# qcraftai/gedepth

Hardware: AMD Instinct MI355X
Metric: training img/s (whole node), KITTI-shaped 352x1120 synthetic batches (higher is better)
Workload: dtype bf16; 1 GPU; depthformer_swint_v: DepthFormer-SwinT + GEDepth-Vanilla, 352x1120, 8 img/GPU, full train step; global_batch=8, parallelism=dp1, allreduce_dtype=fp32, layout=nhwc, window_attention=bf16 mfma, params=53516992, hip_graph=off

## Files before the change

gedepth_amd/csrc/conv1x1_bn.hip:

```cpp
#include "common.h"

#define CB_K 64
#define CB_LD 72
#define CB_GRAM (65 * CB_K)
#define CB_GRAM_WG 256

__device__ __forceinline__ int cb_row(int r, int hi) { return (r & 3) + 8 * (r >> 2) + 4 * hi; }

__global__ void __launch_bounds__(256) conv1x1_gram_k(const bf16_t* __restrict__ x, long rows, float* __restrict__ partial) {
  __shared__ __attribute__((aligned(16))) bf16_t stage_all[4][64 * CB_LD];
  __shared__ float red[CB_GRAM];
  const int lane = threadIdx.x & 63, wv = threadIdx.x >> 6, hi = lane >> 5;
  bf16_t* stage = stage_all[wv];
  ge_f32x16 acc[2][2], sum[2];
#pragma unroll
  for (int i = 0; i < 16; ++i) { acc[0][0][i] = 0.f; acc[0][1][i] = 0.f; acc[1][0][i] = 0.f; acc[1][1][i] = 0.f; sum[0][i] = 0.f; sum[1][i] = 0.f; }
  const ge_bf16x8 ones = {(__bf16)1.f, (__bf16)1.f, (__bf16)1.f, (__bf16)1.f, (__bf16)1.f, (__bf16)1.f, (__bf16)1.f, (__bf16)1.f};
  const int tr_row = hi * 8 + ((lane & 15) >> 2), tr_col = ((lane >> 4) & 1) * 16 + (lane & 3) * 4;
  const long nblk = (rows + 63) / 64;
  for (long blk = (long)blockIdx.x * 4 + wv; blk < nblk; blk += (long)gridDim.x * 4) {
    uint4 R[8];
#pragma unroll
    for (int i = 0; i < 8; ++i) {
      const int idx = i * 64 + lane;
// ... 310 lines not shown
  if (sl == 0) {
    a = (sm[0][j] + sm[1][j]) + (sm[2][j] + sm[3][j]);
    const bf16_t r = f2bf(a);
    Wd[(long)j * (Cout + CB_K) + Cout + i] = r;
    b += (float)(gram[CB_K * CB_K + j] / n) * (a - bf2f(r));
  }
  b = ge_wave_sum(b);
  if (j == 0) sc[sl] = b;
  __syncthreads();
  if (threadIdx.x == 0) c0v[i] = (sc[0] + sc[1]) + (sc[2] + sc[3]);
}

__global__ void __launch_bounds__(256) conv1x1_bn_dgrad_k(const bf16_t* __restrict__ g, const bf16_t* __restrict__ x, const bf16_t* __restrict__ Wd,
                                                          const float* __restrict__ c0, bf16_t* __restrict__ dx, long rows, int Cout) {
  extern __shared__ __attribute__((aligned(16))) bf16_t wl[];
  const int KP = Cout + CB_K, LD = KP + 8, ppr = KP / 8;
  for (int idx = threadIdx.x; idx < CB_K * ppr; idx += 256) {
    const int r = idx / ppr, pc = idx - r * ppr;
    *(uint4*)(wl + r * LD + pc * 8) = *(const uint4*)(Wd + (long)r * KP + pc * 8);
  }
  __syncthreads();
  const int lane = threadIdx.x & 63, wv = threadIdx.x >> 6, hi = lane >> 5, n = lane & 31;
  float c0r[2][16];
#pragma unroll
  for (int mt = 0; mt < 2; ++mt)
#pragma unroll
    for (int r = 0; r < 16; ++r) c0r[mt][r] = c0[mt * 32 + cb_row(r, hi)];
  const bf16_t* wa = wl + n * LD + hi * 8;
  const long ntile = (rows + 31) / 32, tstep = (long)gridDim.x * 4;
  const int nch = Cout / 128;
  ge_bf16x8 Fa[8], Fb[8], Fx[4];
#define CB_ROWPTR(T_) (((T_) * 32 + n < rows) ? (T_) * 32 + n : rows - 1)
#define CB_LOADG(F_, T_, C_) { const bf16_t* gr_ = g + CB_ROWPTR(T_) * Cout + (C_) * 128 + hi * 8; _Pragma("unroll") for (int s_ = 0; s_ < 8; ++s_) F_[s_] = *(const ge_bf16x8*)(gr_ + s_ * 16); }
#define CB_MMA(F_, C_)                                                                                                         \
  _Pragma("unroll") for (int s_ = 0; s_ < 8; ++s_) {                                                                           \
    const ge_bf16x8 w0_ = *(const ge_bf16x8*)(wa + ((C_) * 8 + s_) * 16), w1_ = *(const ge_bf16x8*)(wa + 32 * LD + ((C_) * 8 + s_) * 16); \
    acc0 = __builtin_amdgcn_mfma_f32_32x32x16_bf16(w0_, F_[s_], acc0, 0, 0, 0);                                                 \
    acc1 = __builtin_amdgcn_mfma_f32_32x32x16_bf16(w1_, F_[s_], acc1, 0, 0, 0);                                                 \
  }
  long tile = (long)blockIdx.x * 4 + wv;
  if (tile < ntile) CB_LOADG(Fa, tile, 0)
  for (; tile < ntile; tile += tstep) {
    {
      const bf16_t* xr = x + CB_ROWPTR(tile) * CB_K + hi * 8;
#pragma unroll
      for (int s = 0; s < 4; ++s) Fx[s] = *(const ge_bf16x8*)(xr + s * 16);
    }
    ge_f32x16 acc0, acc1;
#pragma unroll
    for (int i = 0; i < 16; ++i) { acc0[i] = 0.f; acc1[i] = 0.f; }
    for (int c = 0; c < nch; c += 2) {
      if (c + 1 < nch) CB_LOADG(Fb, tile, c + 1)
      CB_MMA(Fa, c)
      if (c + 2 < nch) CB_LOADG(Fa, tile, c + 2)
      else if (tile + tstep < ntile) CB_LOADG(Fa, tile + tstep, 0)
      if (c + 1 < nch) CB_MMA(Fb, c + 1)
    }
#pragma unroll
    for (int s = 0; s < 4; ++s) {
      const ge_bf16x8 w0 = *(const ge_bf16x8*)(wa + Cout + s * 16), w1 = *(const ge_bf16x8*)(wa + 32 * LD + Cout + s * 16);
      acc0 = __builtin_amdgcn_mfma_f32_32x32x16_bf16(w0, Fx[s], acc0, 0, 0, 0);
      acc1 = __builtin_amdgcn_mfma_f32_32x32x16_bf16(w1, Fx[s], acc1, 0, 0, 0);
    }
    const long row = tile * 32 + n;
    if (row < rows) {
      bf16_t* o = dx + row * CB_K + 4 * hi;
#pragma unroll
      for (int r4 = 0; r4 < 4; ++r4) {
        uint2 v0, v1;
        v0.x = ge_pack_bf16x2(acc0[4 * r4] + c0r[0][4 * r4], acc0[4 * r4 + 1] + c0r[0][4 * r4 + 1]);
        v0.y = ge_pack_bf16x2(acc0[4 * r4 + 2] + c0r[0][4 * r4 + 2], acc0[4 * r4 + 3] + c0r[0][4 * r4 + 3]);
        v1.x = ge_pack_bf16x2(acc1[4 * r4] + c0r[1][4 * r4], acc1[4 * r4 + 1] + c0r[1][4 * r4 + 1]);
        v1.y = ge_pack_bf16x2(acc1[4 * r4 + 2] + c0r[1][4 * r4 + 2], acc1[4 * r4 + 3] + c0r[1][4 * r4 + 3]);
        *(uint2*)(o + 8 * r4) = v0;
        *(uint2*)(o + 32 + 8 * r4) = v1;
      }
    }
  }
#undef CB_ROWPTR
#undef CB_LOADG
#undef CB_MMA
}

static inline bool cb_ok(int Cin, int Cout) { return Cin == CB_K && Cout > 0 && Cout % 128 == 0 && Cout <= 2048; }

extern "C" size_t ge_conv1x1_bn_workspace(int Cin, int Cout) {
  if (!cb_ok(Cin, Cout)) return 0;
  const size_t a = (size_t)CB_GRAM_WG * CB_GRAM * sizeof(float), b = (size_t)1024 * Cout * sizeof(float);
  return a > b ? a : b;
}

extern "C" int ge_conv1x1_bn_stats(const void* x, long rows, int Cin, const void* w, int Cout, const float* gamma, const float* beta,
                                   float* running_mean, float* running_var, float eps, float momentum, double* gram, float* save_mean,
                                   float* save_rstd, float* coef, void* workspace, void* stream) {
  if (!x || !w || !gamma || !beta || !gram || !save_mean || !save_rstd || !coef || !workspace || rows <= 0) return GE_ERR_BAD_ARG;
  if (!cb_ok(Cin, Cout) || (((uintptr_t)x | (uintptr_t)w) & 15)) return GE_ERR_UNSUPPORTED;
  hipStream_t s = ge_stream(stream);
  const long nblk = (rows + 63) / 64;
  const int nb = (int)(nblk < 4L * CB_GRAM_WG ? (nblk + 3) / 4 : CB_GRAM_WG);
  conv1x1_gram_k<<<nb, 256, 0, s>>>((const bf16_t*)x, rows, (float*)workspace);
  GE_LAUNCH_CHECK();
  conv1x1_partials_reduce_k<double><<<(CB_GRAM + 31) / 32, 256, 0, s>>>((const float*)workspace, nb, CB_GRAM, gram);
  GE_LAUNCH_CHECK();
  conv1x1_bn_finalize_k<<<(Cout + 3) / 4, 256, 0, s>>>(gram, (const bf16_t*)w, gamma, beta, save_mean, save_rstd, running_mean, running_var, coef,
                                                       Cout, (double)rows, eps, momentum);
  GE_LAUNCH_CHECK();
  return GE_OK;
}

extern "C" int ge_conv1x1_bn_act_fwd(const void* x, const void* w, const float* coef, const float* pos, void* y, void* q, int B, long HW, int Cin,
                                     int Cout, float slope, void* stream) {
  if (!x || !w || !coef || !y || B <= 0 || HW <= 0 || (!pos) != (!q)) return GE_ERR_BAD_ARG;
  if (!cb_ok(Cin, Cout) || (((uintptr_t)x | (uintptr_t)w | (uintptr_t)y | (uintptr_t)q | (uintptr_t)pos) & 15)) return GE_ERR_UNSUPPORTED;
  const int cus = ge_cu_count();
  if (!cus) return GE_ERR_BAD_ARG;
  hipStream_t s = ge_stream(stream);
  const long ntile = ((HW + 31) / 32) * B;
#ifndef CB_WGS_PER_CU
#define CB_WGS_PER_CU 4
#endif
  long gx = (long)cus * CB_WGS_PER_CU;
  if (gx > ntile) gx = ntile;
  gx = (gx + 7) / 8 * 8;
  const dim3 grid((unsigned)gx, (unsigned)((Cout / 128 + 3) / 4));
  if (pos) conv1x1_bn_act_k<true><<<grid, 256, 0, s>>>((const bf16_t*)x, (const bf16_t*)w, coef, pos, (bf16_t*)y, (bf16_t*)q, HW, B, Cout, slope);
  else conv1x1_bn_act_k<false><<<grid, 256, 0, s>>>((const bf16_t*)x, (const bf16_t*)w, coef, nullptr, (bf16_t*)y, nullptr, HW, B, Cout, slope);
  GE_LAUNCH_CHECK();
  return GE_OK;
}

extern "C" int ge_conv1x1_bn_bwd_mask(const void* dy1, long ld1, const void* dy2, long ld2, const void* y, void* g, float* colsum, void* workspace,
                                      long rows, int C, float slope, void* stream) {
  if ((!dy1 && !dy2) || !y || !g || !colsum || !workspace || rows <= 0 || C <= 0) return GE_ERR_BAD_ARG;
  if (C % 8 || C > 2048 || (dy1 && ld1 % 8) || (dy2 && ld2 % 8) || (((uintptr_t)dy1 | (uintptr_t)dy2 | (uintptr_t)y | (uintptr_t)g) & 15)) return GE_ERR_UNSUPPORTED;
  hipStream_t s = ge_stream(stream);
  const int lpr = C / 8;
  if (lpr > 256) return GE_ERR_UNSUPPORTED;
  const int rpi = 256 / lpr;
  const unsigned nb = ge_blocks(rows, rpi * 8, 1024);
  float* part = (float*)workspace;
#define CB_MASK(A_, B_) conv1x1_bn_mask_k<A_, B_><<<nb, 256, 0, s>>>((const bf16_t*)dy1, ld1, (const bf16_t*)dy2, ld2, (const bf16_t*)y, (bf16_t*)g, part, C, rows, lpr, rpi, slope)
  if (dy1 && dy2) CB_MASK(true, true);
  else if (dy1) CB_MASK(true, false);
  else CB_MASK(false, true);
#undef CB_MASK
  GE_LAUNCH_CHECK();
  conv1x1_partials_reduce_k<float><<<(C + 31) / 32, 256, 0, s>>>(part, (int)nb, C, colsum);
  GE_LAUNCH_CHECK();
  return GE_OK;
}

extern "C" int ge_conv1x1_bn_bwd_finalize(const float* GT, const float* colsum, const double* gram, const void* w, const float* gamma,
                                          const float* save_mean, const float* save_rstd, long rows, int Cin, int Cout, float* dgamma, float* dbeta,
                                          float* dW, void* Wd, float* c0, float* scratch, void* stream) {
  if (!GT || !colsum || !gram || !w || !gamma || !save_mean || !save_rstd || !dgamma || !dbeta || !dW || !Wd || !c0 || !scratch || rows <= 0) return GE_ERR_BAD_ARG;
  if (!cb_ok(Cin, Cout)) return GE_ERR_UNSUPPORTED;
  hipStream_t s = ge_stream(stream);
  conv1x1_bn_bwd_finalize_k<<<(Cout + 3) / 4, 256, 0, s>>>(GT, colsum, gram, (const bf16_t*)w, gamma, save_mean, save_rstd, dgamma, dbeta, dW, (bf16_t*)Wd,
                                                           scratch, scratch + Cout, Cout, (double)rows);
  GE_LAUNCH_CHECK();
  conv1x1_bn_bwd_a2_k<<<CB_K, 256, 0, s>>>((const bf16_t*)w, scratch, scratch + Cout, gram, (bf16_t*)Wd, c0, Cout, (double)rows);
  GE_LAUNCH_CHECK();
  return GE_OK;
}

extern "C" int ge_conv1x1_bn_dgrad(const void* g, const void* x, const void* Wd, const float* c0, void* dx, long rows, int Cin, int Cout, void* stream) {
  if (!g || !x || !Wd || !c0 || !dx || rows <= 0) return GE_ERR_BAD_ARG;
  if (!cb_ok(Cin, Cout) || Cout > 1024 || (((uintptr_t)g | (uintptr_t)x | (uintptr_t)Wd | (uintptr_t)dx) & 15)) return GE_ERR_UNSUPPORTED;
  const int cus = ge_cu_count();
  if (!cus) return GE_ERR_BAD_ARG;
  const size_t smem = (size_t)CB_K * (Cout + CB_K + 8) * sizeof(bf16_t);
  static bool attr_set = false;
  if (!attr_set) {
    if (hipFuncSetAttribute((const void*)conv1x1_bn_dgrad_k, hipFuncAttributeMaxDynamicSharedMemorySize, 160 * 1024) != hipSuccess) return GE_ERR_UNSUPPORTED;
    attr_set = true;
  }
  const long ntile = (rows + 31) / 32;
  long wgs = (long)cus * (smem <= 78 * 1024 ? 2 : 1);
  if (wgs > (ntile + 3) / 4) wgs = (ntile + 3) / 4;
  conv1x1_bn_dgrad_k<<<(unsigned)wgs, 256, smem, ge_stream(stream)>>>((const bf16_t*)g, (const bf16_t*)x, (const bf16_t*)Wd, c0, (bf16_t*)dx, rows, Cout);
  GE_LAUNCH_CHECK();
  return GE_OK;
}
```

gedepth_amd/hip.py:

```python
import ctypes
import os
import re

import torch

_HERE = os.path.dirname(os.path.abspath(__file__))
LIB_PATH = os.environ.get('GE_LIB') or os.path.join(_HERE, 'csrc', 'libgedepth_hip.so')
HEADERS = {'SIGNATURES': 'gedepth_hip.h', 'EVAL_SIGNATURES': 'gedepth_eval.h', 'DDAD_SIGNATURES': 'gedepth_ddad.h',
           'CLOUD_SIGNATURES': 'gedepth_cloud.h', 'GROUND_SIGNATURES': 'gedepth_ground.h'}
EXTRA_HEADERS = {'BATCH_SIGNATURES': 'gedepth_batch.h'}
SCENE_HEADERS = {'SCENE_SIGNATURES': 'gedepth_scene.h'}
STRATA_HEADERS = {'STRATA_SIGNATURES': 'gedepth_strata.h'}
GE_F32, GE_BF16 = 0, 1
GE_COLORIZE_VMIN_DATA, GE_COLORIZE_VMAX_DATA, GE_COLORIZE_EQUAL = 1, 2, 4

_SCALARS = {'int': ctypes.c_int, 'long': ctypes.c_long, 'float': ctypes.c_float, 'double': ctypes.c_double, 'size_t': ctypes.c_size_t,
            'uint64_t': ctypes.c_ulonglong, 'unsigned long long': ctypes.c_ulonglong}
_DECL = re.compile(r'\b(int|size_t)\s+(ge_\w+)\s*\(([^()]*)\)\s*;')


def parse_header(text):
    text = re.sub(r'/\*.*?\*/|//[^\n]*', ' ', text, flags=re.S)
    sigs = {}
    for res, name, params in _DECL.findall(text):
        args = []
        for p in ([] if params.strip() == 'void' else params.split(',')):
            if '*' in p:
                args.append(ctypes.c_void_p)
                continue
            ctype = ' '.join(w for w in p.split()[:-1] if w != 'const')
            if ctype not in _SCALARS:
                raise TypeError(f'{name}: parameter "{" ".join(p.split())}" has a type the ctypes binding does not map')
            args.append(_SCALARS[ctype])
        sigs[name] = (_SCALARS[res], args)
    stray = set(re.findall(r'\b(ge_\w+)\s*\(', text)) - set(sigs)
    if stray:
        raise TypeError(f'cannot parse the declaration of {", ".join(sorted(stray))}')
    return sigs


for _table, _header in {**HEADERS, **EXTRA_HEADERS, **SCENE_HEADERS, **STRATA_HEADERS}.items():
    with open(os.path.join(os.path.dirname(_HERE), 'include', _header)) as _fh:
        globals()[_table] = parse_header(_fh.read())

_lib = None


class HipLibraryError(RuntimeError):
    pass


def lib():
    global _lib
    if _lib is None:
        if not os.path.isfile(LIB_PATH):
            raise HipLibraryError(
                f'{LIB_PATH} is missing: the gfx950 HIP kernels are not built. '
                f'Run gedepth_amd/csrc/build.sh (hipcc --offload-arch=gfx950). There is no CPU/eager fallback.')
        handle = ctypes.CDLL(LIB_PATH)
        for table in (*HEADERS, *EXTRA_HEADERS, *SCENE_HEADERS, *STRATA_HEADERS):
            for name, (res, args) in globals()[table].items():
                fn = getattr(handle, name)
                fn.restype, fn.argtypes = res, args
        _lib = handle
        if os.environ.get('GE_MSDA_MODE'):
            handle.ge_msda_mode(int(os.environ['GE_MSDA_MODE']))
    return _lib


def is_built():
    return os.path.isfile(LIB_PATH)


def check(code, what):
    if code != 0:
        raise RuntimeError(f'{what} failed with code {code} '
                           f'({"bad argument" if code == 10001 else "unsupported" if code == 10002 else "hipError_t"})')


def call(name, *args):
    code = getattr(_lib or lib(), name)(*args)
    if code:
        check(code, name)


def dtype_code(t):
    if t.dtype == torch.float32:
        return GE_F32
    if t.dtype == torch.bfloat16:
        return GE_BF16
    raise TypeError(f'gedepth_amd kernels take float32 or bfloat16 tensors, got {t.dtype}')


def ptr(t, dtype=None, name='tensor'):
    if t is None:
        return None
    if not t.is_cuda:
        raise RuntimeError(f'{name}: gedepth_amd ops run on MI355X only; got a {t.device} tensor '
                           '(the CPU oracle lives in oracle/ and is test infrastructure)')
    if not t.is_contiguous():
        raise RuntimeError(f'{name} must be contiguous')
    if dtype is not None and t.dtype != dtype:
        raise TypeError(f'{name} must be {dtype}, got {t.dtype}')
    return t.data_ptr()


def stream():
    return torch.cuda.current_stream().cuda_stream
```

gedepth_amd/kernels.py:

```python
import ctypes
import os

import torch

from . import hip

_f32 = torch.float32


def _c(t):
    return t if t.is_contiguous() else t.contiguous()


class _Profiler:

    def __init__(self):
        self.on, self.records, self.stage_bytes = False, {}, {}

    def enable(self):
        self.on, self.records, self.stage_bytes = True, {}, {}
        hip.lib().ge_msda_bwd_timing(1)

    def disable(self):
        self.on = False
# ... 1423 lines not shown
                hip.ptr(y), hip.ptr(stats[0]), hip.ptr(stats[1]), hip.ptr(running_mean, _f32), hip.ptr(running_var, _f32), hip.ptr(ws), N, C, H * W,
                eps, momentum, slope, hip.dtype_code(x), hip.stream())
        ctx.save_for_backward(x, y, w, stats)
        ctx.slope = slope
        return y

    @staticmethod
    def backward(ctx, dy):
        x, y, w, stats = ctx.saved_tensors
        N, C, H, W = x.shape
        dx = torch.empty_like(x)
        dwb = torch.empty(2, C, device=x.device, dtype=_f32)
        ws = torch.empty(int(hip.lib().ge_nhwc_workspace(C, 2) if ctx.cl else hip.lib().ge_bn_workspace(C)), device=x.device, dtype=torch.uint8)
        if ctx.cl:
            dy = _cl(dy.to(x.dtype))
            _launch(f'bn_act_nhwc_bwd[{N}x{C}x{H}x{W} {_tag(x)}]', 5 * x.numel() * _es(x), 'ge_bn_act_nhwc_bwd', _raw_ptr(dy, 'dy'), None,
                    _raw_ptr(x, 'x'), hip.ptr(w), hip.ptr(y, _f32), hip.ptr(stats[0]), hip.ptr(stats[1]), _raw_ptr(dx, 'dx'), hip.ptr(dwb[0]),
                    hip.ptr(dwb[1]), hip.ptr(ws), N * H * W, C, ctx.slope, hip.dtype_code(x), hip.stream())
            return dx, dwb[0], dwb[1], None, None, None, None, None
        dy = _c(dy.to(x.dtype))
        _launch(f'bn_act_bwd[{N}x{C}x{H}x{W} {_tag(x)}]', 7 * x.numel() * _es(x), 'ge_bn_act_bwd', hip.ptr(dy), hip.ptr(y), hip.ptr(x), hip.ptr(w),
                hip.ptr(stats[0]), hip.ptr(stats[1]), hip.ptr(dx), hip.ptr(dwb[0]), hip.ptr(dwb[1]), hip.ptr(ws), N, C, H * W, ctx.slope,
                hip.dtype_code(x), hip.stream())
        return dx, dwb[0], dwb[1], None, None, None, None, None


def bn_act(x, bn, slope=0.0):
    y = _BNAct.apply(x, bn.weight, bn.bias, bn.running_mean, bn.running_var, float(bn.eps), float(bn.momentum), float(slope))
    bn.num_batches_tracked.add_(1)
    return y


class _Conv1x1BNActPos(torch.autograd.Function):

    @staticmethod
    def forward(ctx, x, weight, gamma, beta, running_mean, running_var, pos_rows, eps, momentum, slope):
        from .mmrt.optim import lowp
        lib = hip.lib()
        B, Cin, H, W = x.shape
        Cout = weight.shape[0]
        HW, rows = H * W, B * H * W
        wc = lowp(weight, torch.bfloat16).detach().reshape(Cout, Cin)
        g32, b32 = _c(gamma.detach().to(_f32)), _c(beta.detach().to(_f32))
        dev = x.device
        ws = torch.empty(int(lib.ge_conv1x1_bn_workspace(Cin, Cout)), device=dev, dtype=torch.uint8)
        gram = torch.empty(65 * Cin, device=dev, dtype=torch.float64)
        stats = torch.empty(2, Cout, device=dev, dtype=_f32)
        coef = torch.empty(2, Cout, device=dev, dtype=_f32)
        y = torch.empty((B, Cout, H, W), device=dev, dtype=x.dtype, memory_format=_CL)
        q = torch.empty(B, HW, Cout, device=dev, dtype=x.dtype) if pos_rows is not None else None
        _launch(f'conv1x1_bn_stats[{B}x{Cin}->{Cout} {H}x{W}]', x.numel() * 2, 'ge_conv1x1_bn_stats', _raw_ptr(x, 'x'), rows, Cin, hip.ptr(wc), Cout,
                hip.ptr(g32), hip.ptr(b32), hip.ptr(running_mean, _f32), hip.ptr(running_var, _f32), eps, momentum, hip.ptr(gram), hip.ptr(stats[0]),
                hip.ptr(stats[1]), hip.ptr(coef), hip.ptr(ws), hip.stream())
        _launch(f'conv1x1_bn_act_fwd[{B}x{Cin}->{Cout} {H}x{W}{" +pos" if q is not None else ""}]',
                x.numel() * 2 + y.numel() * 2 * (1 + (q is not None)) + (HW * Cout * 4 if q is not None else 0), 'ge_conv1x1_bn_act_fwd',
                _raw_ptr(x, 'x'), hip.ptr(wc), hip.ptr(coef), hip.ptr(pos_rows, _f32), _raw_ptr(y, 'y'), hip.ptr(q), B, HW, Cin, Cout, slope,
                hip.stream())
        ctx.save_for_backward(x, wc, g32, stats, gram, y)
        ctx.meta = (slope, weight.dtype, gamma.dtype, beta.dtype)
        ctx.weight_ref = weight if isinstance(weight, torch.nn.Parameter) else None
        if q is None:
            return y
        return y, q

    @staticmethod
    def backward(ctx, dy, dq=None):
        x, wc, g32, stats, gram, y = ctx.saved_tensors
        slope, w_dtype, g_dtype, b_dtype = ctx.meta
        lib = hip.lib()
        B, Cin, H, W = x.shape
        Cout = wc.shape[0]
        rows = B * H * W
        dev = x.device
        ld_y = 0
        if dy is not None:
            dy = dy.to(x.dtype)
            ld_y = dy.stride(3)
            if not (dy.stride(1) == 1 and ld_y >= Cout and ld_y % 8 == 0 and dy.stride(2) == W * ld_y and dy.stride(0) == H * W * ld_y and dy.data_ptr() % 16 == 0):
                dy, ld_y = _cl(dy), Cout
        if dq is not None:
            dq = _c(dq.to(x.dtype))
        if dy is None and dq is None:
            return (None,) * 10
        ws = torch.empty(int(lib.ge_conv1x1_bn_workspace(Cin, Cout)), device=dev, dtype=torch.uint8)
        g = torch.empty(rows, Cout, device=dev, dtype=x.dtype)
        m1 = torch.empty(Cout, device=dev, dtype=_f32)
        _launch(f'conv1x1_bn_bwd_mask[{B}x{Cout} {H}x{W}]', g.numel() * 2 * (2 + (dy is not None) + (dq is not None)), 'ge_conv1x1_bn_bwd_mask',
                hip.ptr(dq), Cout, None if dy is None else _raw_ptr(dy, 'dy'), ld_y, _raw_ptr(y, 'y'), hip.ptr(g), hip.ptr(m1), hip.ptr(ws), rows,
                Cout, slope, hip.stream())
        GT = torch.zeros(Cout, Cin, device=dev, dtype=_f32)
        _launch(f'conv1x1_wgrad[{B}x{Cin}->{Cout} {H}x{W}]', (x.numel() + g.numel()) * 2 + GT.numel() * 4, 'ge_conv1x1_nhwc_wgrad', _raw_ptr(x, 'x'),
                hip.ptr(g), hip.ptr(GT), rows, Cin, Cout, hip.GE_BF16, hip.stream())
        small = torch.empty(2 * Cout + Cout * Cin + 2 * Cout, device=dev, dtype=_f32)
        dgamma, dbeta, dW, scratch = small[:Cout], small[Cout:2 * Cout], small[2 * Cout:2 * Cout + Cout * Cin].view(Cout, Cin), small[2 * Cout + Cout * Cin:]
        Wd = torch.empty(Cin, Cout + Cin, device=dev, dtype=x.dtype)
        c0 = torch.empty(Cin, device=dev, dtype=_f32)
        hip.call('ge_conv1x1_bn_bwd_finalize', hip.ptr(GT), hip.ptr(m1), hip.ptr(gram), hip.ptr(wc), hip.ptr(g32), hip.ptr(stats[0]),
                 hip.ptr(stats[1]), rows, Cin, Cout, hip.ptr(dgamma), hip.ptr(dbeta), hip.ptr(dW), hip.ptr(Wd), hip.ptr(c0), hip.ptr(scratch),
                 hip.stream())
        dx = None
        if ctx.needs_input_grad[0]:
            dx = torch.empty_like(x)
            _launch(f'conv1x1_bn_dgrad[{B}x{Cout}->{Cin} {H}x{W}]', (g.numel() + 2 * x.numel()) * 2, 'ge_conv1x1_bn_dgrad', hip.ptr(g),
                    _raw_ptr(x, 'x'), hip.ptr(Wd), hip.ptr(c0), _raw_ptr(dx, 'dx'), rows, Cin, Cout, hip.stream())
        dw = dW.view(Cout, Cin, 1, 1)
        if ctx.weight_ref is not None:
            from .mmrt.optim import grad_into_arena
            dw = grad_into_arena(ctx.weight_ref, dw, w_dtype)
        else:
            dw = dw.to(w_dtype)
        return dx, dw, dgamma.to(g_dtype), dbeta.to(b_dtype), None, None, None, None, None, None


def conv1x1_bn_act_pos_ok(block, x):
    conv, bn = block.conv, block.norm
    return ('conv1x1_bn' not in DISABLED and x.is_cuda and x.dtype == torch.bfloat16 and type(conv) is torch.nn.Conv2d and conv.kernel_size == (1, 1)
            and conv.stride == (1, 1) and conv.padding == (0, 0) and conv.groups == 1 and conv.bias is None and conv.in_channels == 64
            and conv.out_channels % 128 == 0 and conv.out_channels <= 1024 and conv.weight.dtype == _f32
            and torch.is_autocast_enabled() and torch.get_autocast_dtype('cuda') == torch.bfloat16
            and block._fused_bn_slope() is not None and _is_cl(x) and x.data_ptr() % 16 == 0)


def conv1x1_bn_act_pos(block, x, pos=None):
    bn = block.norm
    slope = float(block._fused_bn_slope())
    pos_rows = _pos_rows(pos) if pos is not None else None
    out = _Conv1x1BNActPos.apply(x, block.conv.weight, bn.weight, bn.bias, bn.running_mean, bn.running_var, pos_rows, float(bn.eps), float(bn.momentum), slope)
    bn.num_batches_tracked.add_(1)
    return out if pos is not None else (out, None)


class _BiasAct(torch.autograd.Function):

    @staticmethod
    def forward(ctx, x, bias, slope):
        ctx.cl = _cl_ok(x)
        assert x.dim() == 4 and (x.is_contiguous() or ctx.cl), 'bias_act works in place on a dense NCHW / channels-last conv output'
        N, C, H, W = x.shape
        b = _c(bias.detach().to(_f32))
        if ctx.cl:
            _launch(f'bias_act_nhwc_fwd[{N}x{C}x{H}x{W} {_tag(x)}]', 2 * x.numel() * _es(x), 'ge_bias_act_nhwc_fwd', _raw_ptr(x, 'x'), hip.ptr(b),
                    N * H * W, C, slope, hip.dtype_code(x), hip.stream())
            ctx.mark_dirty(x)
            ctx.save_for_backward(x)
            ctx.slope = slope
            return x
        _launch(f'bias_act_fwd[{N}x{C}x{H}x{W} {_tag(x)}]', 2 * x.numel() * _es(x), 'ge_bias_act_fwd', hip.ptr(x, name='x'), hip.ptr(b), N, C, H * W,
                slope, hip.dtype_code(x), hip.stream())
        ctx.mark_dirty(x)
        ctx.save_for_backward(x)
        ctx.slope = slope
        return x

    @staticmethod
    def backward(ctx, dy):
        y, = ctx.saved_tensors
        N, C, H, W = y.shape
        dx = torch.empty_like(y)
        if ctx.cl:
            dy = _cl(dy.to(y.dtype))
            db = torch.empty(C, device=y.device, dtype=_f32)
            ws = torch.empty(int(hip.lib().ge_nhwc_workspace(C, 1)), device=y.device, dtype=torch.uint8)
            _launch(f'bias_act_nhwc_bwd[{N}x{C}x{H}x{W} {_tag(y)}]', 3 * y.numel() * _es(y), 'ge_bias_act_nhwc_bwd', _raw_ptr(dy, 'dy'),
                    _raw_ptr(y, 'y'), _raw_ptr(dx, 'dx'), hip.ptr(db), hip.ptr(ws), N * H * W, C, ctx.slope, hip.dtype_code(y), hip.stream())
            return dx, db, None
        dy = _c(dy.to(y.dtype))
        db = torch.zeros(C, device=y.device, dtype=_f32)
        _launch(f'bias_act_bwd[{N}x{C}x{H}x{W} {_tag(y)}]', 3 * y.numel() * _es(y), 'ge_bias_act_bwd', hip.ptr(dy), hip.ptr(y), hip.ptr(dx),
                hip.ptr(db), N, C, H * W, ctx.slope, hip.dtype_code(y), hip.stream())
        return dx, db, None


def bias_act_(conv_out, bias, slope=1.0):
    return _BiasAct.apply(conv_out, bias, float(slope))


def _plane_view(img, channel):
    if not img.is_cuda:
        raise RuntimeError('gedepth_amd ops run on MI355X only; got a CPU image tensor')
    assert img.dim() == 4 and img.is_contiguous() and img.dtype == _f32
    return img[:, channel], img.stride(0)


class _GroundEmbedAdaptive(torch.autograd.Function):
# ... 257 lines not shown
```

Measured before the change: 170.4 img/s.

## Fuse conv1x1+BN backward mask, wgrad and partial dgrad into one pass

Adds a single-pass backward kernel for the 64-channel 1x1 conv+BN+leaky block. It applies the activation mask to dy in registers, accumulates the weight gradient from LDS, and computes a partial dgrad product P in the same pass, so the bf16 intermediate g (rows x Cout) is never written to or reread from global memory. A small second kernel adds the x-dependent term and writes dx. The new path is used only for large activations with Cout<=512. In exchange it writes an fp32 P buffer and uses atomics for GT, and it rounds the gamma*rstd-scaled weight to bf16, which may shift numerics slightly.

Result: no change. 171.4 img/s (median of 6 runs) (+0.6%).

```diff
diff --git a/gedepth_amd/csrc/conv1x1_bn.hip b/gedepth_amd/csrc/conv1x1_bn.hip
--- a/gedepth_amd/csrc/conv1x1_bn.hip
+++ b/gedepth_amd/csrc/conv1x1_bn.hip
@@ -416,6 +416,205 @@
 #undef CB_MMA
 }
 
+#define CB_GLD 136
+#define CB_OP_LDS(COUT_) ((size_t)(CB_K * ((COUT_) + 8) + 2 * 128 * CB_GLD + 128 * CB_LD) * sizeof(bf16_t))
+
+template <bool ONE, bool TWO>
+__device__ __forceinline__ uint32_t cb_mask2(uint32_t a, uint32_t b, uint32_t yv, float slope) {
+  float lo = (ONE ? __uint_as_float(a << 16) : 0.f) + (TWO ? __uint_as_float(b << 16) : 0.f);
+  float up = (ONE ? __uint_as_float(a & 0xffff0000u) : 0.f) + (TWO ? __uint_as_float(b & 0xffff0000u) : 0.f);
+  lo = __uint_as_float(yv << 16) > 0.f ? lo : lo * slope;
+  up = __uint_as_float(yv & 0xffff0000u) > 0.f ? up : up * slope;
+  return (uint32_t)f2bf(lo) | ((uint32_t)f2bf(up) << 16);
+}
+
+template <int NCH, bool ONE, bool TWO>
+__global__ void __launch_bounds__(256) conv1x1_bn_bwd_onepass_k(const bf16_t* dy1, long ld1, const bf16_t* dy2, long ld2, const bf16_t* y, const bf16_t* x,
+                                                                const bf16_t* __restrict__ w, const float* __restrict__ gamma,
+                                                                const float* __restrict__ save_rstd, float slope, long rows, float* __restrict__ P,
+                                                                float* __restrict__ GT, float* __restrict__ partial, bf16_t* __restrict__ a1_dbg) {
+  constexpr int Cout = NCH * 128, LD = Cout + 8;
+  extern __shared__ __attribute__((aligned(16))) bf16_t cb_sm[];
+  bf16_t* a1 = cb_sm;
+  bf16_t* gs = a1 + CB_K * LD;
+  bf16_t* xs = gs + 2 * 128 * CB_GLD;
+  for (int idx = threadIdx.x; idx < Cout * CB_K; idx += 256) {
+    const int c = idx >> 6, i = idx & 63;
+    const double a = (double)gamma[c] * (double)save_rstd[c];
+    const bf16_t v = f2bf((float)(a * (double)bf2f(w[idx])));
+    a1[i * LD + c] = v;
+    if (a1_dbg && blockIdx.x == 0) a1_dbg[(long)i * Cout + c] = v;
+  }
+  const int lane = threadIdx.x & 63, wv = threadIdx.x >> 6, hi = lane >> 5, n = lane & 31;
+  const int tr_row = hi * 8 + ((lane & 15) >> 2), tr_col = ((lane >> 4) & 1) * 16 + (lane & 3) * 4;
+  const bf16_t* wa = a1 + n * LD + hi * 8;
+  const long nblk = (rows + 127) / 128;
+  ge_f32x16 accG[NCH][2];
+  float cs[NCH];
+#pragma unroll
+  for (int c = 0; c < NCH; ++c) {
+    cs[c] = 0.f;
+#pragma unroll
+    for (int i = 0; i < 16; ++i) { accG[c][0][i] = 0.f; accG[c][1][i] = 0.f; }
+  }
+  uint4 R1[8], R2[8], RY[8], RX[4];
+  const uint4 zero4 = make_uint4(0, 0, 0, 0);
+#pragma unroll
+  for (int s = 0; s < 8; ++s) { R1[s] = zero4; R2[s] = zero4; }
+#define CB_OP_ROW(B_) (((B_) * 128 + wv * 32 + n < rows) ? (B_) * 128 + wv * 32 + n : rows - 1)
+#define CB_OP_LOAD(S_, B_, C_)                                                                             \
+  {                                                                                                        \
+    const long r_ = CB_OP_ROW(B_);                                                                         \
+    const int o_ = (C_) * 128 + hi * 8 + (S_) * 16;                                                        \
+    if (ONE) R1[S_] = *(const uint4*)(dy1 + r_ * ld1 + o_);                                                \
+    if (TWO) R2[S_] = *(const uint4*)(dy2 + r_ * ld2 + o_);                                                \
+    RY[S_] = *(const uint4*)(y + r_ * Cout + o_);                                                          \
+  }
+#define CB_OP_LOADX(B_)                                                                                    \
+  _Pragma("unroll") for (int i_ = 0; i_ < 4; ++i_) {                                                       \
+    const int idx_ = i_ * 64 + lane;                                                                       \
+    const long r_ = (B_) * 128 + wv * 32 + (idx_ >> 3);                                                    \
+    RX[i_] = *(const uint4*)(x + (r_ < rows ? r_ : rows - 1) * CB_K + (idx_ & 7) * 8);                     \
+  }
+  long blk = blockIdx.x;
+#pragma unroll
+  for (int s = 0; s < 8; ++s) CB_OP_LOAD(s, blk, 0)
+  CB_OP_LOADX(blk)
+  for (; blk < nblk; blk += gridDim.x) {
+    const long row = blk * 128 + wv * 32 + n, nxt = blk + gridDim.x;
+    const bool valid = row < rows;
+    const uint32_t vmask = valid ? 0xffffffffu : 0u;
+    __syncthreads();
+#pragma unroll
+    for (int i = 0; i < 4; ++i) {
+      const int idx = i * 64 + lane, tok = wv * 32 + (idx >> 3);
+      const uint32_t keep = blk * 128 + tok < rows ? 0xffffffffu : 0u;
+      *(uint4*)(xs + tok * CB_LD + (idx & 7) * 8) = make_uint4(RX[i].x & keep, RX[i].y & keep, RX[i].z & keep, RX[i].w & keep);
+    }
+    CB_OP_LOADX(nxt)
+    ge_f32x16 acc0, acc1;
+#pragma unroll
+    for (int i = 0; i < 16; ++i) { acc0[i] = 0.f; acc1[i] = 0.f; }
+#pragma unroll
+    for (int c = 0; c < NCH; ++c) {
+      bf16_t* gb = gs + (c & 1) * 128 * CB_GLD;
+#pragma unroll
+      for (int s = 0; s < 8; ++s) {
+        if (ONE) asm volatile("" : "+v"(R1[s].x), "+v"(R1[s].y), "+v"(R1[s].z), "+v"(R1[s].w));
+        if (TWO) asm volatile("" : "+v"(R2[s].x), "+v"(R2[s].y), "+v"(R2[s].z), "+v"(R2[s].w));
+        asm volatile("" : "+v"(RY[s].x), "+v"(RY[s].y), "+v"(RY[s].z), "+v"(RY[s].w));
+        uint4 F;
+        F.x = cb_mask2<ONE, TWO>(R1[s].x, R2[s].x, RY[s].x, slope) & vmask;
+        F.y = cb_mask2<ONE, TWO>(R1[s].y, R2[s].y, RY[s].y, slope) & vmask;
+        F.z = cb_mask2<ONE, TWO>(R1[s].z, R2[s].z, RY[s].z, slope) & vmask;
+        F.w = cb_mask2<ONE, TWO>(R1[s].w, R2[s].w, RY[s].w, slope) & vmask;
+        if (c + 1 < NCH) CB_OP_LOAD(s, blk, c + 1)
+        else CB_OP_LOAD(s, nxt, 0)
+        *(uint4*)(gb + (wv * 32 + n) * CB_GLD + s * 16 + hi * 8) = F;
+        const ge_bf16x8 f = __builtin_bit_cast(ge_bf16x8, F);
+        const ge_bf16x8 w0 = *(const ge_bf16x8*)(wa + (c * 8 + s) * 16), w1 = *(const ge_bf16x8*)(wa + 32 * LD + (c * 8 + s) * 16);
+        acc0 = __builtin_amdgcn_mfma_f32_32x32x16_bf16(w0, f, acc0, 0, 0, 0);
+        acc1 = __builtin_amdgcn_mfma_f32_32x32x16_bf16(w1, f, acc1, 0, 0, 0);
+      }
+      __syncthreads();
+#pragma unroll
+      for (int ks = 0; ks < 8; ++ks) {
+        const bf16_t* pg = gb + (ks * 16 + tr_row) * CB_GLD + wv * 32 + tr_col;
+        const bf16_t* px = xs + (ks * 16 + tr_row) * CB_LD + tr_col;
+        const ge_bf16x4 g0 = __builtin_amdgcn_ds_read_tr16_b64_v4bf16(GE_LDS(ge_bf16x4, pg));
+        const ge_bf16x4 g1 = __builtin_amdgcn_ds_read_tr16_b64_v4bf16(GE_LDS(ge_bf16x4, pg + 4 * CB_GLD));
+        const ge_bf16x4 x00 = __builtin_amdgcn_ds_read_tr16_b64_v4bf16(GE_LDS(ge_bf16x4, px));
+        const ge_bf16x4 x01 = __builtin_amdgcn_ds_read_tr16_b64_v4bf16(GE_LDS(ge_bf16x4, px + 4 * CB_LD));
+        const ge_bf16x4 x10 = __builtin_amdgcn_ds_read_tr16_b64_v4bf16(GE_LDS(ge_bf16x4, px + 32));
+        const ge_bf16x4 x11 = __builtin_amdgcn_ds_read_tr16_b64_v4bf16(GE_LDS(ge_bf16x4, px + 32 + 4 * CB_LD));
+        const ge_bf16x8 A = __builtin_shufflevector(g0, g1, 0, 1, 2, 3, 4, 5, 6, 7);
+        accG[c][0] = __builtin_amdgcn_mfma_f32_32x32x16_bf16(A, __builtin_shufflevector(x00, x01, 0, 1, 2, 3, 4, 5, 6, 7), accG[c][0], 0, 0, 0);
+        accG[c][1] = __builtin_amdgcn_mfma_f32_32x32x16_bf16(A, __builtin_shufflevector(x10, x11, 0, 1, 2, 3, 4, 5, 6, 7), accG[c][1], 0, 0, 0);
+        const uint4 au = __builtin_bit_cast(uint4, A);
+        cs[c] += ((__uint_as_float(au.x << 16) + __uint_as_float(au.x & 0xffff0000u)) + (__uint_as_float(au.y << 16) + __uint_as_float(au.y & 0xffff0000u))) +
+                 ((__uint_as_float(au.z << 16) + __uint_as_float(au.z & 0xffff0000u)) + (__uint_as_float(au.w << 16) + __uint_as_float(au.w & 0xffff0000u)));
+      }
+    }
+    if (valid) {
+      float* o = P + row * CB_K + 4 * hi;
+#pragma unroll
+      for (int r4 = 0; r4 < 4; ++r4) {
+        *(float4*)(o + 8 * r4) = make_float4(acc0[4 * r4], acc0[4 * r4 + 1], acc0[4 * r4 + 2], acc0[4 * r4 + 3]);
+        *(float4*)(o + 32 + 8 * r4) = make_float4(acc1[4 * r4], acc1[4 * r4 + 1], acc1[4 * r4 + 2], acc1[4 * r4 + 3]);
+      }
+    }
+  }
+#undef CB_OP_ROW
+#undef CB_OP_LOAD
+#undef CB_OP_LOADX
+#pragma unroll
+  for (int c = 0; c < NCH; ++c) {
+#pragma unroll
+    for (int b = 0; b < 2; ++b)
+#pragma unroll
+      for (int r = 0; r < 16; ++r) atomicAdd(GT + (long)(c * 128 + wv * 32 + cb_row(r, hi)) * CB_K + b * 32 + n, accG[c][b][r]);
+    const float s = cs[c] + __shfl_xor(cs[c], 32, 64);
+    if (hi == 0) partial[(long)blockIdx.x * Cout + c * 128 + wv * 32 + n] = s;
+  }
+}
+
+__global__ void __launch_bounds__(256) conv1x1_bn_bwd_dx_k(const float* __restrict__ P, const bf16_t* __restrict__ x, const bf16_t* __restrict__ Wd,
+                                                           const float* __restrict__ c0, bf16_t* __restrict__ dx, long rows, int Cout) {
+  __shared__ __attribute__((aligned(16))) bf16_t a2[CB_K * CB_LD];
+  const int KP = Cout + CB_K;
+  for (int idx = threadIdx.x; idx < CB_K * 8; idx += 256) {
+    const int r = idx >> 3, pc = idx & 7;
+    *(uint4*)(a2 + r * CB_LD + pc * 8) = *(const uint4*)(Wd + (long)r * KP + Cout + pc * 8);
+  }
+  __syncthreads();
+  const int lane = threadIdx.x & 63, wv = threadIdx.x >> 6, hi = lane >> 5, n = lane & 31;
+  float c0r[2][16];
+  ge_bf16x8 W0[4], W1[4];
+#pragma unroll
+  for (int mt = 0; mt < 2; ++mt)
+#pragma unroll
+    for (int r = 0; r < 16; ++r) c0r[mt][r] = c0[mt * 32 + cb_row(r, hi)];
+#pragma unroll
+  for (int s = 0; s < 4; ++s) {
+    W0[s] = *(const ge_bf16x8*)(a2 + n * CB_LD + hi * 8 + s * 16);
+    W1[s] = *(const ge_bf16x8*)(a2 + (32 + n) * CB_LD + hi * 8 + s * 16);
+  }
+  const long ntile = (rows + 31) / 32;
+  for (long tile = (long)blockIdx.x * 4 + wv; tile < ntile; tile += (long)gridDim.x * 4) {
+    const long row = tile * 32 + n, rc = row < rows ? row : rows - 1;
+    ge_bf16x8 Fx[4];
+    ge_f32x16 acc0, acc1;
+    const bf16_t* xr = x + rc * CB_K + hi * 8;
+    const float* pr = P + rc * CB_K + 4 * hi;
+#pragma unroll
+    for (int s = 0; s < 4; ++s) Fx[s] = *(const ge_bf16x8*)(xr + s * 16);
+#pragma unroll
+    for (int r4 = 0; r4 < 4; ++r4) {
+      const float4 p0 = *(const float4*)(pr + 8 * r4), p1 = *(const float4*)(pr + 32 + 8 * r4);
+      acc0[4 * r4] = p0.x; acc0[4 * r4 + 1] = p0.y; acc0[4 * r4 + 2] = p0.z; acc0[4 * r4 + 3] = p0.w;
+      acc1[4 * r4] = p1.x; acc1[4 * r4 + 1] = p1.y; acc1[4 * r4 + 2] = p1.z; acc1[4 * r4 + 3] = p1.w;
+    }
+#pragma unroll
+    for (int s = 0; s < 4; ++s) {
+      acc0 = __builtin_amdgcn_mfma_f32_32x32x16_bf16(W0[s], Fx[s], acc0, 0, 0, 0);
+      acc1 = __builtin_amdgcn_mfma_f32_32x32x16_bf16(W1[s], Fx[s], acc1, 0, 0, 0);
+    }
+    if (row < rows) {
+      bf16_t* o = dx + row * CB_K + 4 * hi;
+#pragma unroll
+      for (int r4 = 0; r4 < 4; ++r4) {
+        uint2 v0, v1;
+        v0.x = ge_pack_bf16x2(acc0[4 * r4] + c0r[0][4 * r4], acc0[4 * r4 + 1] + c0r[0][4 * r4 + 1]);
+        v0.y = ge_pack_bf16x2(acc0[4 * r4 + 2] + c0r[0][4 * r4 + 2], acc0[4 * r4 + 3] + c0r[0][4 * r4 + 3]);
+        v1.x = ge_pack_bf16x2(acc1[4 * r4] + c0r[1][4 * r4], acc1[4 * r4 + 1] + c0r[1][4 * r4 + 1]);
+        v1.y = ge_pack_bf16x2(acc1[4 * r4 + 2] + c0r[1][4 * r4 + 2], acc1[4 * r4 + 3] + c0r[1][4 * r4 + 3]);
+        *(uint2*)(o + 8 * r4) = v0;
+        *(uint2*)(o + 32 + 8 * r4) = v1;
+      }
+    }
+  }
+}
+
 static inline bool cb_ok(int Cin, int Cout) { return Cin == CB_K && Cout > 0 && Cout % 128 == 0 && Cout <= 2048; }
 
 extern "C" size_t ge_conv1x1_bn_workspace(int Cin, int Cout) {
@@ -516,3 +715,58 @@
   GE_LAUNCH_CHECK();
   return GE_OK;
 }
+
+#include "../../include/gedepth_neck.h"
+#define CB_OP_MAX_WG 1024
+static inline bool cb_op_ok(int Cin, int Cout) { return cb_ok(Cin, Cout) && Cout <= 512; }
+
+extern "C" size_t ge_conv1x1_bn_bwd_onepass_workspace(int Cin, int Cout) {
+  return cb_op_ok(Cin, Cout) ? (size_t)CB_OP_MAX_WG * Cout * sizeof(float) : 0;
+}
+
+typedef void (*cb_onepass_fn)(const bf16_t*, long, const bf16_t*, long, const bf16_t*, const bf16_t*, const bf16_t*, const float*, const float*, float, long,
+                              float*, float*, float*, bf16_t*);
+#define CB_OP_ROUTES(N_) {conv1x1_bn_bwd_onepass_k<N_, true, true>, conv1x1_bn_bwd_onepass_k<N_, true, false>, conv1x1_bn_bwd_onepass_k<N_, false, true>}
+
+extern "C" int ge_conv1x1_bn_bwd_onepass(const void* dy1, long ld1, const void* dy2, long ld2, const void* y, const void* x, const void* w,
+                                         const float* gamma, const float* save_rstd, float slope, long rows, int Cin, int Cout, float* P, float* GT,
+                                         float* colsum, void* workspace, void* a1_debug, void* stream) {
+  if ((!dy1 && !dy2) || !y || !x || !w || !gamma || !save_rstd || !P || !GT || !colsum || !workspace || rows <= 0) return GE_ERR_BAD_ARG;
+  if (!cb_op_ok(Cin, Cout) || (dy1 && (ld1 % 8 || ld1 < Cout)) || (dy2 && (ld2 % 8 || ld2 < Cout)) ||
+      (((uintptr_t)dy1 | (uintptr_t)dy2 | (uintptr_t)y | (uintptr_t)x | (uintptr_t)P) & 15))
+    return GE_ERR_UNSUPPORTED;
+  const int cus = ge_cu_count();
+  if (!cus) return GE_ERR_BAD_ARG;
+  static const cb_onepass_fn table[4][3] = {CB_OP_ROUTES(1), CB_OP_ROUTES(2), CB_OP_ROUTES(3), CB_OP_ROUTES(4)};
+  static bool attr_set[4][3] = {};
+  const int nch = Cout / 128 - 1, route = dy1 && dy2 ? 0 : dy1 ? 1 : 2;
+  const cb_onepass_fn fn = table[nch][route];
+  const size_t smem = CB_OP_LDS(Cout);
+  if (!attr_set[nch][route]) {
+    if (hipFuncSetAttribute((const void*)fn, hipFuncAttributeMaxDynamicSharedMemorySize, 160 * 1024) != hipSuccess) return GE_ERR_UNSUPPORTED;
+    attr_set[nch][route] = true;
+  }
+  hipStream_t s = ge_stream(stream);
+  const long nblk = (rows + 127) / 128;
+  long wgs = cus < CB_OP_MAX_WG ? cus : CB_OP_MAX_WG;
+  if (wgs > nblk) wgs = nblk;
+  fn<<<(unsigned)wgs, 256, smem, s>>>((const bf16_t*)dy1, ld1, (const bf16_t*)dy2, ld2, (const bf16_t*)y, (const bf16_t*)x, (const bf16_t*)w, gamma, save_rstd,
+                                      slope, rows, P, GT, (float*)workspace, (bf16_t*)a1_debug);
+  GE_LAUNCH_CHECK();
+  conv1x1_partials_reduce_k<float><<<(Cout + 31) / 32, 256, 0, s>>>((const float*)workspace, (int)wgs, Cout, colsum);
+  GE_LAUNCH_CHECK();
+  return GE_OK;
+}
+
+extern "C" int ge_conv1x1_bn_bwd_dx(const float* P, const void* x, const void* Wd, const float* c0, void* dx, long rows, int Cin, int Cout, void* stream) {
+  if (!P || !x || !Wd || !c0 || !dx || rows <= 0) return GE_ERR_BAD_ARG;
+  if (!cb_ok(Cin, Cout) || (((uintptr_t)P | (uintptr_t)x | (uintptr_t)Wd | (uintptr_t)dx) & 15)) return GE_ERR_UNSUPPORTED;
+  const int cus = ge_cu_count();
+  if (!cus) return GE_ERR_BAD_ARG;
+  const long ntile = (rows + 31) / 32;
+  long wgs = (long)cus * 3;
+  if (wgs > (ntile + 3) / 4) wgs = (ntile + 3) / 4;
+  conv1x1_bn_bwd_dx_k<<<(unsigned)wgs, 256, 0, ge_stream(stream)>>>(P, (const bf16_t*)x, (const bf16_t*)Wd, c0, (bf16_t*)dx, rows, Cout);
+  GE_LAUNCH_CHECK();
+  return GE_OK;
+}
diff --git a/gedepth_amd/hip.py b/gedepth_amd/hip.py
--- a/gedepth_amd/hip.py
+++ b/gedepth_amd/hip.py
@@ -11,6 +11,7 @@
 EXTRA_HEADERS = {'BATCH_SIGNATURES': 'gedepth_batch.h'}
 SCENE_HEADERS = {'SCENE_SIGNATURES': 'gedepth_scene.h'}
 STRATA_HEADERS = {'STRATA_SIGNATURES': 'gedepth_strata.h'}
+NECK_HEADERS = {'NECK_SIGNATURES': 'gedepth_neck.h'}
 GE_F32, GE_BF16 = 0, 1
 GE_COLORIZE_VMIN_DATA, GE_COLORIZE_VMAX_DATA, GE_COLORIZE_EQUAL = 1, 2, 4
 
@@ -39,7 +40,7 @@
     return sigs
 
 
-for _table, _header in {**HEADERS, **EXTRA_HEADERS, **SCENE_HEADERS, **STRATA_HEADERS}.items():
+for _table, _header in {**HEADERS, **EXTRA_HEADERS, **SCENE_HEADERS, **STRATA_HEADERS, **NECK_HEADERS}.items():
     with open(os.path.join(os.path.dirname(_HERE), 'include', _header)) as _fh:
         globals()[_table] = parse_header(_fh.read())
 
@@ -58,7 +59,7 @@
                 f'{LIB_PATH} is missing: the gfx950 HIP kernels are not built. '
                 f'Run gedepth_amd/csrc/build.sh (hipcc --offload-arch=gfx950). There is no CPU/eager fallback.')
         handle = ctypes.CDLL(LIB_PATH)
-        for table in (*HEADERS, *EXTRA_HEADERS, *SCENE_HEADERS, *STRATA_HEADERS):
+        for table in (*HEADERS, *EXTRA_HEADERS, *SCENE_HEADERS, *STRATA_HEADERS, *NECK_HEADERS):
             for name, (res, args) in globals()[table].items():
                 fn = getattr(handle, name)
                 fn.restype, fn.argtypes = res, args
diff --git a/gedepth_amd/kernels.py b/gedepth_amd/kernels.py
--- a/gedepth_amd/kernels.py
+++ b/gedepth_amd/kernels.py
@@ -1529,15 +1529,20 @@
             dq = _c(dq.to(x.dtype))
         if dy is None and dq is None:
             return (None,) * 10
-        ws = torch.empty(int(lib.ge_conv1x1_bn_workspace(Cin, Cout)), device=dev, dtype=torch.uint8)
-        g = torch.empty(rows, Cout, device=dev, dtype=x.dtype)
-        m1 = torch.empty(Cout, device=dev, dtype=_f32)
-        _launch(f'conv1x1_bn_bwd_mask[{B}x{Cout} {H}x{W}]', g.numel() * 2 * (2 + (dy is not None) + (dq is not None)), 'ge_conv1x1_bn_bwd_mask',
-                hip.ptr(dq), Cout, None if dy is None else _raw_ptr(dy, 'dy'), ld_y, _raw_ptr(y, 'y'), hip.ptr(g), hip.ptr(m1), hip.ptr(ws), rows,
-                Cout, slope, hip.stream())
-        GT = torch.zeros(Cout, Cin, device=dev, dtype=_f32)
-        _launch(f'conv1x1_wgrad[{B}x{Cin}->{Cout} {H}x{W}]', (x.numel() + g.numel()) * 2 + GT.numel() * 4, 'ge_conv1x1_nhwc_wgrad', _raw_ptr(x, 'x'),
-                hip.ptr(g), hip.ptr(GT), rows, Cin, Cout, hip.GE_BF16, hip.stream())
+        from . import neck_kernels as NK
+        onepass = NK.conv1x1_bn_bwd_onepass_ok(rows, Cin, Cout)
+        if onepass:
+            P, GT, m1 = NK.conv1x1_bn_bwd_onepass(dq, dy, ld_y, y, x, wc, g32, stats[1], slope, (B, Cin, H, W, Cout))
+        else:
+            ws = torch.empty(int(lib.ge_conv1x1_bn_workspace(Cin, Cout)), device=dev, dtype=torch.uint8)
+            g = torch.empty(rows, Cout, device=dev, dtype=x.dtype)
+            m1 = torch.empty(Cout, device=dev, dtype=_f32)
+            _launch(f'conv1x1_bn_bwd_mask[{B}x{Cout} {H}x{W}]', g.numel() * 2 * (2 + (dy is not None) + (dq is not None)), 'ge_conv1x1_bn_bwd_mask',
+                    hip.ptr(dq), Cout, None if dy is None else _raw_ptr(dy, 'dy'), ld_y, _raw_ptr(y, 'y'), hip.ptr(g), hip.ptr(m1), hip.ptr(ws), rows,
+                    Cout, slope, hip.stream())
+            GT = torch.zeros(Cout, Cin, device=dev, dtype=_f32)
+            _launch(f'conv1x1_wgrad[{B}x{Cin}->{Cout} {H}x{W}]', (x.numel() + g.numel()) * 2 + GT.numel() * 4, 'ge_conv1x1_nhwc_wgrad', _raw_ptr(x, 'x'),
+                    hip.ptr(g), hip.ptr(GT), rows, Cin, Cout, hip.GE_BF16, hip.stream())
         small = torch.empty(2 * Cout + Cout * Cin + 2 * Cout, device=dev, dtype=_f32)
         dgamma, dbeta, dW, scratch = small[:Cout], small[Cout:2 * Cout], small[2 * Cout:2 * Cout + Cout * Cin].view(Cout, Cin), small[2 * Cout + Cout * Cin:]
         Wd = torch.empty(Cin, Cout + Cin, device=dev, dtype=x.dtype)
@@ -1546,7 +1551,9 @@
                  hip.ptr(stats[1]), rows, Cin, Cout, hip.ptr(dgamma), hip.ptr(dbeta), hip.ptr(dW), hip.ptr(Wd), hip.ptr(c0), hip.ptr(scratch),
                  hip.stream())
         dx = None
-        if ctx.needs_input_grad[0]:
+        if ctx.needs_input_grad[0] and onepass:
+            dx = NK.conv1x1_bn_bwd_dx(P, x, Wd, c0, Cout)
+        elif ctx.needs_input_grad[0]:
             dx = torch.empty_like(x)
             _launch(f'conv1x1_bn_dgrad[{B}x{Cout}->{Cin} {H}x{W}]', (g.numel() + 2 * x.numel()) * 2, 'ge_conv1x1_bn_dgrad', hip.ptr(g),
                     _raw_ptr(x, 'x'), hip.ptr(Wd), hip.ptr(c0), _raw_ptr(dx, 'dx'), rows, Cin, Cout, hip.stream())
diff --git a/gedepth_amd/neck_kernels.py b/gedepth_amd/neck_kernels.py
--- /dev/null
+++ b/gedepth_amd/neck_kernels.py
@@ -0,0 +1,36 @@
+import torch
+
+from . import hip
+
+ONEPASS_MIN_BYTES = 64 << 20
+
+
+def conv1x1_bn_bwd_onepass_ok(rows, Cin, Cout):
+    from . import kernels
+    return ('conv1x1_bn_onepass' not in kernels.DISABLED and rows * Cout * 2 >= ONEPASS_MIN_BYTES
+            and hip.lib().ge_conv1x1_bn_bwd_onepass_workspace(Cin, Cout) > 0)
+
+
+def conv1x1_bn_bwd_onepass(dq, dy, ld_y, y, x, wc, gamma, rstd, slope, shape, a1_debug=None):
+    from .kernels import _launch, _raw_ptr
+    B, Cin, H, W, Cout = shape
+    rows, dev = B * H * W, x.device
+    ws = torch.empty(int(hip.lib().ge_conv1x1_bn_bwd_onepass_workspace(Cin, Cout)), device=dev, dtype=torch.uint8)
+    P = torch.empty(rows, Cin, device=dev, dtype=torch.float32)
+    GT = torch.zeros(Cout, Cin, device=dev, dtype=torch.float32)
+    m1 = torch.empty(Cout, device=dev, dtype=torch.float32)
+    nbytes = rows * Cout * 2 * (1 + (dy is not None) + (dq is not None)) + rows * Cin * (2 + 4) + GT.numel() * 4
+    _launch(f'conv1x1_bn_bwd_onepass[{B}x{Cout} {H}x{W}]', nbytes, 'ge_conv1x1_bn_bwd_onepass', hip.ptr(dq), Cout,
+            None if dy is None else _raw_ptr(dy, 'dy'), ld_y, _raw_ptr(y, 'y'), _raw_ptr(x, 'x'), hip.ptr(wc), hip.ptr(gamma), hip.ptr(rstd),
+            slope, rows, Cin, Cout, hip.ptr(P), hip.ptr(GT), hip.ptr(m1), hip.ptr(ws), hip.ptr(a1_debug), hip.stream(),
+            flops=2 * 2 * rows * Cout * Cin)
+    return P, GT, m1
+
+
+def conv1x1_bn_bwd_dx(P, x, Wd, c0, Cout):
+    from .kernels import _launch, _raw_ptr
+    B, Cin, H, W = x.shape
+    dx = torch.empty_like(x)
+    _launch(f'conv1x1_bn_bwd_dx[{B}x{Cout}->{Cin} {H}x{W}]', P.numel() * 4 + 2 * x.numel() * 2, 'ge_conv1x1_bn_bwd_dx', hip.ptr(P), _raw_ptr(x, 'x'),
+            hip.ptr(Wd), hip.ptr(c0), _raw_ptr(dx, 'dx'), B * H * W, Cin, Cout, hip.stream())
+    return dx
diff --git a/include/gedepth_neck.h b/include/gedepth_neck.h
--- /dev/null
+++ b/include/gedepth_neck.h
@@ -0,0 +1,22 @@
+#ifndef GEDEPTH_NECK_H
+#define GEDEPTH_NECK_H
+
+#include <stddef.h>
+#include <stdint.h>
+
+#ifdef __cplusplus
+extern "C" {
+#endif
+
+size_t ge_conv1x1_bn_bwd_onepass_workspace(int Cin, int Cout);
+
+int ge_conv1x1_bn_bwd_onepass(const void* dy1, long ld1, const void* dy2, long ld2, const void* y, const void* x, const void* w,
+                              const float* gamma, const float* save_rstd, float slope, long rows, int Cin, int Cout, float* P, float* GT,
+                              float* colsum, void* workspace, void* a1_debug, void* stream);
+
+int ge_conv1x1_bn_bwd_dx(const float* P, const void* x, const void* Wd, const float* c0, void* dx, long rows, int Cin, int Cout, void* stream);
+
+#ifdef __cplusplus
+}
+#endif
+#endif
```
